# acerbilab/vbmc

Measured on AMD Instinct MI355X. Metric: ELBO+grad evals/sec (Ns=1e4, K=50, D=10, N=400), higher is better.
Workload: dtype f64; 1 GPU; BASELINE configs[2]: D=10 N=400 K=50 Ns=10000/component S=20, R=64 restarts batched per GPU per step, value+gradient, beta=0, no variance; restarts_per_gpu=64, parallelism=one GPU

## Files before the change

vbmc_amd/csrc/entropy_mfma.h:

```cpp
#pragma once
#include <type_traits>

#include "device_math.h"
#include "elbo_types.h"
#include "exp2_tab1k.h"
#include "logjoint_body.h"

typedef double mf4 __attribute__((ext_vector_type(4)));
struct EntTileAny { static constexpr bool rt = false, val = true; };
struct EntTileFull { static constexpr bool rt = false, val = false; };
struct EntTilePartial { static constexpr bool rt = false, val = true; };
#define VBMC_ENT_SPLIT(KT_, QS_, TL_, HV_) ((HV_) == 1)

#ifdef VBMC_INSTRUMENT
#define VBMC_DBG_WAVES 32768
__device__ unsigned long long g_ent_dbg[6 * VBMC_DBG_WAVES];
#endif

#define VBMC_STAG_FOR(KT_, QS_, TL_) ((KT_) == 1 || (KT_) == 4 || ((KT_) == 2 && (QS_) >= 6) || ((KT_) == 3 && (QS_) <= ((TL_) ? 5 : 8)))



constexpr bool ent_c2_for(int KT, int QS, int TL, int HV) {
  if (HV == 1) {
    if (KT == 2) return !(TL == 1 && QS >= 6);
    if (KT == 3) return QS <= 5 || (TL == 0 && QS != 7) || (TL == 1 && QS == 7);
    if (KT == 4) return QS >= 5;
    return true;
  }
  if (HV == 2) {
    if (KT == 2) return TL != 2;
    if (KT == 3) return !((TL == 1 && (QS == 5 || QS == 6)) || (TL == 2 && QS == 6));
    return true;
  }
  if (KT == 2) return !((TL == 1 && QS >= 6) || (TL == 2 && QS >= 5));
  if (KT == 3) return !(TL == 1 && QS == 7);
  return QS != 5;
}
constexpr bool ent_gp2_for(int KT, int QS, int TL, int HV) { return !(HV == 1 && KT == 1 && TL == 0 && QS <= 3); }
constexpr bool ent_sl_for(int KT, int QS, int TL, int HV, bool GRAD, bool WALK) {
  if (!(GRAD && HV == 1 && QS <= 3) || KT == 4 || WALK) return false;
  if (QS == 3) return !((KT == 1 && TL == 0) || (KT == 2 && TL <= 1));
  if (QS == 2) return KT == 3 || (KT == 2 && TL == 0);
  return TL == 0 || (KT == 2 && TL == 1) || (KT == 3 && TL == 2);
}
constexpr bool ent_sl_evl_for(int KT, int QS, int TL) { return QS == 3 && KT == 3 && TL == 0; }

template <int HV>
__device__ __forceinline__ void ent_sync() {
  __builtin_amdgcn_fence(__ATOMIC_RELEASE, "wavefront");
  __builtin_amdgcn_wave_barrier();
  __builtin_amdgcn_fence(__ATOMIC_ACQUIRE, "wavefront");
}
template <int HV>
__device__ __forceinline__ void ent_sync_wg() {
  if (HV == 1) ent_sync<1>();
  else __syncthreads();
}

template <int QS, int KT, bool GRAD, bool SPARSE, int HV = 1, int TL = 0, bool CO = false, bool EM = true, bool WALK = false>
#define VBMC_ENT_EO(HV_) true
#define VBMC_ENT_ONE_WAVE(KT_, QS_, TL_, HV_) \
  (((HV_) == 1 && (KT_) == 4 && (QS_) >= 5) || ((HV_) == 1 && (KT_) == 3 && (QS_) >= 8) || ((HV_) == 4 && (KT_) == 4 && (QS_) >= 6) || \
   ((HV_) == 4 && (KT_) == 3 && (QS_) >= 9))
#define VBMC_ENT_WAVES(KT_, QS_, TL_, HV_) \
  (VBMC_ENT_ONE_WAVE(KT_, QS_, TL_, HV_) ? 1 : ((((KT_) <= 2 && (QS_) <= 4) && !((KT_) == 2 && (TL_) == 2 && (HV_) == 1)) ? 3 : 2))
__device__ __forceinline__ void ent_mfma_segment(const EntArgs& a, const int c, const int j, const int r, const int t0, const int t1,
                                                 const int pdone, const int ptot) {
  static_assert(!CO || (HV == 1 && QS <= 8 && !SPARSE), "the log-joint role exists for single-wave dense kernels at D <= 30");
  static_assert(!WALK || (HV == 1 && !CO), "the walk exists for single-wave workgroups without the log-joint role");
  static_assert(KT <= 4 && (HV == 1 || HV == 2 || HV == 4 || HV == 8), "larger mixtures are split over the waves of a workgroup (HV = 2, 4; round 5: 8, K <= 512)");
  static_assert(TL == 0 || ((TL == 1 || TL == 2) && !SPARSE), "the component tail (one or two values per lane) exists for the dense kernels only");
  constexpr int TLN = TL > 0 ? TL : 1;
  constexpr bool SP = SPARSE;
  constexpr int DP = 4 * QS;
  constexpr int NPV = (4 * QS + 15) / 16;
  constexpr int QL = QS;
  __shared__ double Et[16 * DP];
  constexpr bool SL = NPV == 1 && ent_sl_for(KT, QS, TL, HV, GRAD, WALK);
  constexpr bool GP2 = GRAD && !SL && ent_gp2_for(KT, QS, TL, HV);
  __shared__ double RQ_all[HV][SL ? 1 : (GP2 ? 32 : 16)];
  __shared__ double BND_all[HV][SPARSE ? KT * 16 * 3 : 1];
  constexpr int YXN = NPV * 4 * WAVE;
  constexpr bool EO = VBMC_ENT_EO(HV);
  constexpr bool YXSB = HV > 1 && EO;
  constexpr bool US = EO;
  constexpr bool VBL = GRAD && HV == 1 && (KT >= 3 || NPV >= 2);
  __shared__ double VBS_all[HV][VBL ? KT * 4 * NPV * WAVE : 1];
  constexpr bool C2 = EO && !SPARSE && ent_c2_for(KT, QS, TL, HV);
#define ENT_CI(kt_, rr_) (16 * (kt_) + 4 * (rr_) + lg)
  __shared__ __attribute__((aligned(16))) double SCP_all[HV][C2 ? KT * 16 * 2 : 2];
  __shared__ double BTL_all[HV][TL ? 4 * TL * DP : 1];
  constexpr bool NML = HV > 1 && EO;
  __shared__ double NMS_all[HV][NML ? KT * 4 * WAVE : 1];
#ifdef VBMC_INSTRUMENT
  const unsigned long long wckE = wall_clock64();
#endif
  int tid_ = threadIdx.x;
  if (WALK) asm volatile("" : "+v"(tid_));
  const int tid = tid_, wv = tid >> 6, hv = HV == 1 ? 0 : wv, lane = tid & 63;
  const int li = lane & 15, lg = lane >> 4;
  int D_ = a.D, K_ = a.K;
  const double *entp_ = a.entp, *vpd_ = a.vpd;
  double* part_ = a.part;
  if (WALK) asm volatile("" : "+s"(D_), "+s"(K_), "+s"(entp_), "+s"(vpd_), "+s"(part_));
  const int D = D_, K = K_;
  double* RQ = RQ_all[wv];
  double* NMS = NMS_all[wv];
  double* BND = BND_all[hv];
  double* VBS = VBS_all[hv];
  double* BTL = BTL_all[hv];
  double* SCP = SCP_all[hv];
  const int Kh = (K + HV - 1) / HV;
  const int kbase = hv * Kh;
  const int Kw = min(K, kbase + Kh) - kbase;
  const int PSg = D + ENTP_EXTRA;
  extern __shared__ double PB[];
  double* const TAB = PB;
  double* const YX = PB + VB_EXP_TAB1K_N;
  constexpr int NTH0 = WAVE * HV;
  constexpr int NTB0 = (VB_EXP_TAB1K_N + NTH0 - 1) / NTH0;
  double tt[NTB0];
#pragma unroll
  for (int u = 0; u < NTB0; ++u) tt[u] = c_exp2_tab1k[min(tid + u * NTH0, VB_EXP_TAB1K_N - 1)];
  const double sigj = vpd_[(size_t)r * VpLayout{D, K}.stride() + VpLayout{D, K}.sigma() + j];
  {
    const double* gsrc = entp_ + (size_t)r * K * PSg;
    constexpr int NT = WAVE * HV;
    const int n = K * PSg;
    int idx = tid;
    for (; idx + 7 * NT < n; idx += 8 * NT) {
      double t8[8];
#pragma unroll
      for (int u = 0; u < 8; ++u) t8[u] = gsrc[idx + u * NT];
#pragma unroll
      for (int u = 0; u < 8; ++u) PB[idx + u * NT] = t8[u];
    }
    {
      double t8[8];
#pragma unroll
      for (int u = 0; u < 8; ++u) t8[u] = (idx + u * NT < n) ? gsrc[idx + u * NT] : 0.0;
#pragma unroll
      for (int u = 0; u < 8; ++u) if (idx + u * NT < n) PB[idx + u * NT] = t8[u];
    }
  }
  __syncthreads();
  const double* gp = PB;
  const double* pj = gp + (size_t)j * PSg;
  const double cKj = pj[D + 1];
  const double hj_neg = 0.5 / (sigj * sigj);
  const int nr_last = TL ? 4 : max(1, min(4, (Kw - 16 * (KT - 1) + 3) >> 2));
  constexpr unsigned FULL_MASK = (1u << KT) - 1u;
  const double logwj = SPARSE ? log(pj[D + 2]) : 0.0;

  constexpr double ESC = VB_EXP_TAB1K_SCALE;
  double SA[KT][QL];
  double SC[KT];
  double VB[VBL ? 1 : KT][4][NPV];
  double WF[KT][4];
#pragma unroll
  for (int kt = 0; kt < KT; ++kt) {
    const int k = 16 * kt + li;
    const bool kv = k < Kw;
    const double* pk = gp + (size_t)(kv ? kbase + k : 0) * PSg;
    double h = pk[D];
    double m2 = 0.0;
    for (int d = 0; d < D; ++d) { double t = pk[d] - pj[d]; m2 = fma(t, t, m2); }
    if (SPARSE && lg == 0) {
      BND[(16 * kt + li) * 3 + 0] = sqrt(m2);
      BND[(16 * kt + li) * 3 + 1] = kv ? pk[D + 1] - cKj : -1.0e30;
      BND[(16 * kt + li) * 3 + 2] = h;
    }
#pragma unroll
    for (int q = 0; q < QL; ++q) {
      const int cc = 4 * q + lg;
      if (EO) {
        double sav = (kv && cc < D) ? ESC * (-2.0 * h * (pk[cc] - pj[cc])) : 0.0;
        if (C2) {
          if (cc == D) sav = kv ? ESC * (h + hj_neg) : 0.0;
          if (cc == D + 1) sav = ESC * (kv ? fma(h, m2, pk[D + 1]) - cKj : -1.0e6);
        }
        SA[kt][q] = sav;
      } else {
        double v;
        if (!kv) v = (cc == D + 1) ? -1.0e6 : 0.0;
        else if (cc < D) v = -2.0 * h * (pk[cc] - pj[cc]);
        else if (cc == D) v = h + hj_neg;
        else if (cc == D + 1) v = fma(h, m2, pk[D + 1]) - cKj;
        else v = 0.0;
        SA[kt][q] = ESC * v;
      }
    }
    SC[kt] = ESC * (!kv ? (lg == 1 ? -1.0e6 : 0.0)
                        : (lg == 0 ? h + hj_neg : (lg == 1 ? fma(h, m2, pk[D + 1]) - cKj : 0.0)));
    if (C2 && lg < 2) SCP[(16 * kt + li) * 2 + lg] = 2.0 * SC[kt];
#pragma unroll
    for (int rr = 0; rr < 4; ++rr) {
      const int k2 = ENT_CI(kt, rr);
      const bool kv2 = k2 < Kw;
      const double* p2 = gp + (size_t)(kv2 ? kbase + k2 : 0) * PSg;
      if (GRAD) {
#pragma unroll
        for (int pv = 0; pv < NPV; ++pv) {
          const int col = 16 * pv + li;
          double v = 0.0;
          if (SL) {
            if (kv2) {
              if (li >= 12) v = p2[D + 2];
              else if (li >= 10) v = p2[D + 3];
              else if (li < D) v = p2[D + 3] * (p2[li] - pj[li]);
            }
          } else
          if (kv2) {
            if (col == 0) v = p2[D + 2];
            else if (col == 1) v = p2[D + 3];
            else if (col < 2 + D) v = p2[D + 3] * (p2[col - 2] - pj[col - 2]);
          }
          if (VBL) VBS[((kt * 4 + rr) * NPV + pv) * WAVE + lane] = v;
          else VB[VBL ? 0 : kt][rr][pv] = v;
        }
      } else {
        WF[kt][rr] = kv2 ? p2[D + 2] : 0.0;
      }
    }
  }

  double tC0[TLN], tC1[TLN], VBt[TLN][NPV], WFt[TLN], Wt[TLN];
#pragma unroll
  for (int u = 0; u < TLN; ++u) {
    tC0[u] = 0.0; tC1[u] = 0.0; WFt[u] = 0.0; Wt[u] = 0.0;
#pragma unroll
    for (int pv = 0; pv < NPV; ++pv) VBt[u][pv] = 0.0;
  }
  if (TL) {
#pragma unroll
    for (int u = 0; u < TLN; ++u) {
      const int tq = 4 * u + lg;
      const int kq = 16 * KT + tq;
      const bool kvq = kq < Kw;
      const double* pq = gp + (size_t)(kvq ? kbase + kq : 0) * PSg;
      const double h = pq[D];
      double m2 = 0.0;
      for (int d = 0; d < D; ++d) { double t = pq[d] - pj[d]; m2 = fma(t, t, m2); }
      tC0[u] = kvq ? ESC * (h + hj_neg) : 0.0;
      tC1[u] = ESC * (kvq ? fma(h, m2, pq[D + 1]) - cKj : -1.0e6);
      for (int d = li; d < DP; d += 16) BTL[tq * DP + d] = (kvq && d < D) ? ESC * (-2.0 * h * (pq[d] - pj[d])) : 0.0;
      if (GRAD) {
#pragma unroll
        for (int pv = 0; pv < NPV; ++pv) {
          const int col = 16 * pv + li;
          double v = 0.0;
          if (SL) {
            if (kvq) {
              if (li >= 12) v = pq[D + 2];
              else if (li >= 10) v = pq[D + 3];
              else if (li < D) v = pq[D + 3] * (pq[li] - pj[li]);
            }
          } else
          if (kvq) {
            if (col == 0) v = pq[D + 2];
            else if (col == 1) v = pq[D + 3];
            else if (col < 2 + D) v = pq[D + 3] * (pq[col - 2] - pj[col - 2]);
          }
          VBt[u][pv] = v;
        }
      } else {
        WFt[u] = kvq ? pq[D + 2] : 0.0;
      }
    }
  }

  __syncthreads();
  {
#pragma unroll
    for (int u = 0; u < NTB0; ++u) if (VB_EXP_TAB1K_N % NTH0 == 0 || tid + u * NTH0 < VB_EXP_TAB1K_N) TAB[tid + u * NTH0] = tt[u];
  }
  __syncthreads();

#define SAV(kt_, q_) SA[kt_][q_]
  constexpr int VBR = (VBL && NPV == 1 && HV == 1 && KT == 3 && !CO) ? ((EM && QS <= 4) ? (TL == 2 ? 4 : 10) : 12) : 0;
  double VBreg[VBR > 0 ? VBR : 1];
#pragma unroll
  for (int u = 0; u < VBR; ++u) VBreg[u] = VBS[u * WAVE + lane];
#define VBV(kt_, rr_, pv_) (VBL ? (((kt_) * 4 + (rr_)) * NPV + (pv_) < VBR ? VBreg[(((kt_) * 4 + (rr_)) * NPV + (pv_)) < VBR ? (((kt_) * 4 + (rr_)) * NPV + (pv_)) : 0] : VBS[(((kt_) * 4 + (rr_)) * NPV + (pv_)) * WAVE + lane]) : VB[VBL ? 0 : (kt_)][rr_][pv_])
  constexpr int NG = SL ? QS : NPV;
  double accH = 0.0, accG[NG], accLG[NG];
  double pm = 1.0;
  int pe = 0, pcnt = 0;
  double Wacc[KT][4];
#pragma unroll
  for (int pv = 0; pv < NG; ++pv) { accG[pv] = 0.0; accLG[pv] = 0.0; }
#pragma unroll
  for (int kt = 0; kt < KT; ++kt)
#pragma unroll
    for (int rr = 0; rr < 4; ++rr) Wacc[kt][rr] = 0.0;

#ifdef VBMC_INSTRUMENT
  const unsigned long long wck0 = wall_clock64();
#endif
  const int ntile = (a.Mh + 15) >> 4;
  const double sfm0 = lg == 0 ? 1.0 : 0.0, sfm1 = lg == 1 ? 1.0 : 0.0;
  const int emask = (4 * (QS - 1) + lg < D) ? -1 : 0;
  const int emask2 = (QS >= 2 && 4 * (QS - 2) + lg < D) ? -1 : 0;
  const double* epsr = a.eps ? a.eps + (size_t)r * a.eps_stride_r + (size_t)j * a.Mh * D : nullptr;
  constexpr bool EPF = EM && HV == 1 && QS <= 4 && KT <= 3 && !SPARSE;
  double epre[EPF ? QS : 1];
  auto eps_fetch = [&](const int tile) {
#pragma unroll
    for (int u = 0; u < (EPF ? QS : 0); ++u) {
      const int idx = lane + u * WAVE, i = idx / DP, d = idx - i * DP;
      double v = 0.0;
      if (tile < t1 && d < D && tile * 16 + i < a.Mh) v = epsr[(size_t)(tile * 16 + i) * D + d];
      epre[u] = v;
    }
  };
  if (EPF && epsr) eps_fetch(t0);
  if (!epsr && (HV == 1 || hv == 0))
    for (int idx = lane; idx < 16 * DP; idx += WAVE) Et[idx] = 0.0;
  const int evm1 = emask, evm2 = emask2;
  const double c2u1 = (4 * (QS - 1) + lg == D) ? 1.0 : 0.0, c2o1 = (4 * (QS - 1) + lg == D + 1) ? 1.0 : 0.0;
  const double c2u2 = (QS >= 2 && 4 * (QS - 2) + lg == D) ? 1.0 : 0.0;

  auto tile_body = [&](const int tile, auto pkind) __attribute__((always_inline)) {
    using PK = decltype(pkind);
    const int b0 = tile * 16;
    ent_sync_wg<HV>();
    if (HV > 1 && hv != 0) {
    } else if (EPF && epsr) {
#pragma unroll
      for (int u = 0; u < (EPF ? QS : 0); ++u) Et[lane + u * WAVE] = US ? sigj * epre[u] : epre[u];
      eps_fetch(tile + 1);
    } else if (epsr) {
      for (int idx = lane; idx < 16 * DP; idx += WAVE) {
        const int i = idx / DP, d = idx - i * DP;
        Et[idx] = (d < D && b0 + i < a.Mh) ? (US ? sigj * epsr[(size_t)(b0 + i) * D + d] : epsr[(size_t)(b0 + i) * D + d]) : 0.0;
      }
    } else {
      unsigned long long seed_t = a.seed;
      if (WALK) asm volatile("" : "+s"(seed_t));
#pragma unroll
      for (int q = lg; q < QS; q += 4) {
        double z4[4] = {0.0, 0.0, 0.0, 0.0};
#define VBMC_RNG_CALL_FOR(KT_, QS_, TL_, HV_) ((HV_) == 2 && (((KT_) == 2 && (TL_) == 2 && (QS_) == 5) || ((KT_) == 3 && (TL_) == 0 && (QS_) == 7)))
        if constexpr (!VBMC_RNG_CALL_FOR(KT, QS, TL, HV)) {
        if (q < (D + 3) / 4) { const vb_d4 zz = vb_normal4i(seed_t, (unsigned)(b0 + li), (unsigned)j, (unsigned)(a.r0 + r * a.rstride), (unsigned)q); z4[0] = zz[0]; z4[1] = zz[1]; z4[2] = zz[2]; z4[3] = zz[3]; }
        } else {
        if (q < (D + 3) / 4) vb_normal4(seed_t, (unsigned)(b0 + li), (unsigned)j, (unsigned)(a.r0 + r * a.rstride), (unsigned)q, z4);
        }
#undef VBMC_RNG_CALL_FOR
        if (q < (D + 3) / 4) {
#pragma unroll
        for (int t = 0; t < 4; ++t) Et[li * DP + 4 * q + t] = US ? sigj * z4[t] : z4[t];
        }
      }
    }
    ent_sync_wg<HV>();
    double ev[QS];
    double e2 = 0.0;
#pragma unroll
    for (int q = 0; q < QS; ++q) {
      ev[q] = Et[li * DP + 4 * q + lg];
      if (q == QS - 1) ev[q] = __hiloint2double(__double2hiint(ev[q]) & evm1, __double2loint(ev[q]) & evm1);
      if (QS >= 2 && q == QS - 2) ev[q] = __hiloint2double(__double2hiint(ev[q]) & evm2, __double2loint(ev[q]) & evm2);
      e2 = fma(ev[q], ev[q], e2);
    }
    e2 = xor_sum16(e2);
    e2 = xor_sum32(e2);
    double shift = US ? fma(-e2, hj_neg, cKj) : cKj - 0.5 * e2;
    const double u2 = US ? e2 : sigj * sigj * e2;
    if (US && SPARSE) e2 *= 2.0 * hj_neg;
    constexpr bool partial = PK::val;
    const bool svalid = b0 + li < a.Mh;
    if (partial) shift = svalid ? shift : 0.0;
    unsigned act = FULL_MASK;
    if (SPARSE) {
      double e2m = e2;
      e2m = fmax(e2m, __shfl_xor(e2m, 1, 64)); e2m = fmax(e2m, __shfl_xor(e2m, 2, 64));
      e2m = fmax(e2m, __shfl_xor(e2m, 4, 64)); e2m = fmax(e2m, __shfl_xor(e2m, 8, 64));
      const double umax = sigj * sqrt(e2m);
      const double own = 0.5 * e2m - logwj;
      act = 0u;
#pragma unroll
      for (int kt = 0; kt < KT; ++kt) {
        const double* bk = BND + (16 * kt + li) * 3;
        const double t = fmax(0.0, bk[0] - umax);
        const double bnd = fma(bk[2] * t, t, bk[1]) + own;
        if (__any(bnd > -a.cutoff)) act |= 1u << kt;
      }
    }

    mf4 n[KT], nm[(EO && !NML) ? KT : 1];
    if (EO) {
      const double sfc = fma(u2, sfm0, sfm1);
      double sfl[QL];
#pragma unroll
      for (int q = 0; q < QL; ++q) sfl[q] = US ? ev[q] : ev[q] * sigj;
      if (C2) {
        sfl[QL - 1] = fma(u2, c2u1, sfl[QL - 1] + c2o1);
        if (QS >= 2) sfl[QL >= 2 ? QL - 2 : 0] = fma(u2, c2u2, sfl[QL >= 2 ? QL - 2 : 0]);
      }
#pragma unroll
      for (int kt = 0; kt < KT; ++kt) {
        n[kt] = (mf4){0.0, 0.0, 0.0, 0.0};
        if (!NML) nm[(EO && !NML) ? kt : 0] = (mf4){0.0, 0.0, 0.0, 0.0};
        if (C2) {
#pragma unroll
          for (int q = 0; q < QL; ++q) n[kt] = __builtin_amdgcn_mfma_f64_16x16x4f64(SAV(kt, q), sfl[q], n[kt], 0, 0, 0);
          mf4 e2nd;
#pragma unroll
          for (int rr = 0; rr < 4; ++rr) {
            const double2 pr = *reinterpret_cast<const double2*>(SCP + ENT_CI(kt, rr) * 2);
            e2nd[rr] = fma(pr.x, u2, pr.y) - n[kt][rr];
          }
          if (NML) {
#pragma unroll
            for (int rr = 0; rr < 4; ++rr) NMS[(kt * 4 + rr) * WAVE + lane] = e2nd[rr];
          } else {
            nm[(EO && !NML) ? kt : 0] = e2nd;
          }
        } else
        if (!SP || ((act >> kt) & 1u)) {
          const mf4 cacc = __builtin_amdgcn_mfma_f64_16x16x4f64(SC[kt], sfc, n[kt], 0, 0, 0);
          n[kt] = cacc;
#pragma unroll
          for (int q = 0; q < QL; ++q)
            n[kt] = __builtin_amdgcn_mfma_f64_16x16x4f64(SAV(kt, q), sfl[q], n[kt], 0, 0, 0);
          if (NML) {
            const mf4 e2nd = 2.0 * cacc - n[kt];
#pragma unroll
            for (int rr = 0; rr < 4; ++rr) NMS[(kt * 4 + rr) * WAVE + lane] = e2nd[rr];
          } else {
            nm[(EO && !NML) ? kt : 0] = 2.0 * cacc - n[kt];
          }
        }
      }
    }

    double ntl[TLN], ntm[TLN];
#pragma unroll
    for (int u = 0; u < TLN; ++u) { ntl[u] = 0.0; ntm[u] = 0.0; }
    if (TL) {
#pragma unroll
      for (int u = 0; u < TLN; ++u) {
        double lt = 0.0;
#pragma unroll
        for (int d = 0; d < DP; ++d) lt = fma(BTL[(4 * u + lg) * DP + d], Et[li * DP + d], lt);
        if (!US) lt *= sigj;
        const double ct = fma(tC0[u], u2, tC1[u]);
        ntl[u] = ct + lt;
        ntm[u] = ct - lt;
      }
    }

    auto exps = [&](mf4 (&x)[KT], auto k0c, auto k1c) {
      constexpr int k0 = decltype(k0c)::value, k1 = decltype(k1c)::value;
#pragma unroll
      for (int kt = k0; kt < k1; ++kt) {
        if (kt < KT - 1) {
          if (!SP || ((act >> kt) & 1u)) x[kt] = vb_exp_tab1k4<VB_EXP_TAB1K_QUAD>(x[kt], TAB);
          else x[kt] = (mf4){0.0, 0.0, 0.0, 0.0};
        } else if (SP && !((act >> (KT - 1)) & 1u)) {
          x[KT - 1] = (mf4){0.0, 0.0, 0.0, 0.0};
        } else if (nr_last == 4) {
          x[KT - 1] = vb_exp_tab1k4<VB_EXP_TAB1K_QUAD>(x[KT - 1], TAB);
        } else {
          mf4 t = x[KT - 1];
          x[KT - 1] = (mf4){0.0, 0.0, 0.0, 0.0};
          x[KT - 1][0] = vb_exp_tab1k<VB_EXP_TAB1K_QUAD>(t[0], TAB);
          if (nr_last > 1) x[KT - 1][1] = vb_exp_tab1k<VB_EXP_TAB1K_QUAD>(t[1], TAB);
          if (nr_last > 2) x[KT - 1][2] = vb_exp_tab1k<VB_EXP_TAB1K_QUAD>(t[2], TAB);
        }
      }
    };
    auto texp = [&](double (&t)[TLN]) {
      if (TL) {
#pragma unroll
        for (int u = 0; u < TLN; ++u) t[u] = vb_exp_tab1k<VB_EXP_TAB1K_QUAD>(t[u], TAB);
      }
    };
    auto pvstep = [&](mf4 (&x)[KT], mf4 (&Y)[NPV], int sg, const double (&tn)[TLN]) {
      constexpr bool TWO = NPV == 1 && KT <= 2;
      auto pvm = [&](double xa, double vb, mf4 acc) __attribute__((always_inline)) {
        return SL ? __builtin_amdgcn_mfma_f64_16x16x4f64(vb, xa, acc, 0, 0, 0) : __builtin_amdgcn_mfma_f64_16x16x4f64(xa, vb, acc, 0, 0, 0);
      };
      mf4 Y2s[TWO ? NPV : 1];
      mf4 (&Y2)[TWO ? NPV : 1] = Y2s;
#pragma unroll
      for (int pv = 0; pv < NPV; ++pv) { Y[pv] = (mf4){0.0, 0.0, 0.0, 0.0}; if (TWO) Y2[pv] = (mf4){0.0, 0.0, 0.0, 0.0}; }
#pragma unroll
      for (int kt = 0; kt < KT - 1; ++kt) {
        if (SP && !((act >> kt) & 1u)) continue;
#pragma unroll
        for (int pv = 0; pv < NPV; ++pv) {
          mf4& Yb = TWO ? Y2[TWO ? pv : 0] : Y[pv];
          Y[pv] = pvm(x[kt][0], VBV(kt, 0, pv), Y[pv]);
          Yb = pvm(x[kt][1], VBV(kt, 1, pv), Yb);
          Y[pv] = pvm(x[kt][2], VBV(kt, 2, pv), Y[pv]);
          Yb = pvm(x[kt][3], VBV(kt, 3, pv), Yb);
        }
      }
#pragma unroll
      for (int pv = 0; pv < NPV; ++pv) {
        mf4& Yb = TWO ? Y2[TWO ? pv : 0] : Y[pv];
        if (SP && !((act >> (KT - 1)) & 1u)) { if (TWO) Y[pv] += Yb; continue; }
        Y[pv] = pvm(x[KT - 1][0], VBV(KT - 1, 0, pv), Y[pv]);
        if (nr_last > 1) Yb = pvm(x[KT - 1][1], VBV(KT - 1, 1, pv), Yb);
        if (nr_last > 2) Y[pv] = pvm(x[KT - 1][2], VBV(KT - 1, 2, pv), Y[pv]);
        if (nr_last > 3) Yb = pvm(x[KT - 1][3], VBV(KT - 1, 3, pv), Yb);
        if (TL) {
#pragma unroll
          for (int u = 0; u < TLN; ++u) Y[pv] = pvm(tn[u], VBt[u][pv], Y[pv]);
        }
        if (TWO) Y[pv] += Yb;
      }
      if (HV > 1) {
        if (YXSB && sg == 1) __syncthreads();
#pragma unroll
        for (int pv = 0; pv < NPV; ++pv)
#pragma unroll
          for (int rr = 0; rr < 4; ++rr) YX[((YXSB ? 0 : sg) * HV + hv) * YXN + (pv * 4 + rr) * WAVE + lane] = Y[pv][rr];
        __syncthreads();
#pragma unroll
        for (int pv = 0; pv < NPV; ++pv)
#pragma unroll
          for (int rr = 0; rr < 4; ++rr) {
            double t = YX[((YXSB ? 0 : sg) * HV + 0) * YXN + (pv * 4 + rr) * WAVE + lane];
#pragma unroll
            for (int w = 1; w < HV; ++w) t += YX[((YXSB ? 0 : sg) * HV + w) * YXN + (pv * 4 + rr) * WAVE + lane];
            Y[pv][rr] = t;
          }
      }
    };
    auto put_q = [&](mf4 (&Y)[NPV]) {
      if constexpr (SL) return;
      if (GP2 ? li < 2 : li == 0) {
#pragma unroll
        for (int rr = 0; rr < 4; ++rr) RQ[(GP2 ? 16 * li : 0) + lg + 4 * rr] = Y[0][rr];
      }
      ent_sync<HV>();
    };
    double arq = 0.0;
    constexpr bool TQ = GP2 && US && NPV == 1 && HV == 1 && EO && KT == 3 && QS <= 3 && !CO && !EM && VBMC_STAG_FOR(KT, QS, TL);
    double tq[TQ ? 4 : 1];
    auto get_rq = [&](mf4 (&Y)[NPV]) -> double {
      double qs_ = SL ? Y[0][3] : RQ[li];
      double rqs = vb_rcp(qs_);
      if (partial) {
        qs_ = svalid ? qs_ : 1.0;
        rqs = svalid ? rqs : 0.0;
      }
      if (GP2) arq = RQ[GP2 ? 16 + li : 0] * rqs;
      if (SL) {
        const double t = Y[0][2] * rqs;
        const auto lo = __builtin_amdgcn_permlane32_swap((unsigned)__double2loint(t), (unsigned)__double2loint(t), false, false);
        const auto hi = __builtin_amdgcn_permlane32_swap((unsigned)__double2hiint(t), (unsigned)__double2hiint(t), false, false);
        arq = __hiloint2double((int)hi[1], (int)lo[1]);
      }
      pm *= __builtin_amdgcn_frexp_mant(qs_);
      pe += __builtin_amdgcn_frexp_exp(qs_);
      accH += shift;
      return rqs;
    };
    auto wacc = [&](mf4 (&x)[KT], double rqs, const double (&tn)[TLN]) {
      if (TL) {
#pragma unroll
        for (int u = 0; u < TLN; ++u) Wt[u] = fma(tn[u], rqs, Wt[u]);
      }
#pragma unroll
      for (int kt = 0; kt < KT; ++kt) {
        if (SP && !((act >> kt) & 1u)) continue;
#pragma unroll
        for (int rr = 0; rr < 4; ++rr) Wacc[kt][rr] = fma(x[kt][rr], rqs, Wacc[kt][rr]);
      }
    };
    auto put_rq = [&](double rqs) {
      if constexpr (SL) return;
      ent_sync<HV>();
      if (lg == 0) { RQ[li] = rqs; if (GP2) RQ[GP2 ? 16 + li : 0] = arq; }
      ent_sync<HV>();
    };
    auto gradpieces = [&](mf4 (&Y)[NPV], double rqs, double ssig, auto sgc) {
      constexpr int SG = decltype(sgc)::value;
      constexpr bool EVL = SL && ent_sl_evl_for(KT, QS, TL);
      int eo = li * DP + lg;
      if (EVL) asm volatile("" : "+v"(eo));
      if constexpr (SL) {
#pragma unroll
        for (int r = 0; r < QS; ++r) {
          const double tv = EVL ? Et[eo + 4 * r] : ev[r];
          const double t = (US && SG > 0) ? tv : ((US && SG < 0) ? -tv : ssig * tv);
          const double gd = fma(t, arq, -(Y[0][r] * rqs));
          accG[r] += gd;
          accLG[r] = fma(t, gd, accLG[r]);
        }
        return;
      }
      if constexpr (GP2) {
#pragma unroll
        for (int rr = 0; rr < 4; ++rr) {
          const int i = lg + 4 * rr;
          const double rq = RQ[i], ar = RQ[GP2 ? 16 + i : 0];
#pragma unroll
          for (int pv = 0; pv < NPV; ++pv) {
            if (HV > 1 && (pv % HV) != hv) continue;
            const int d = min(max(16 * pv + li - 2, 0), DP - 1);
            double tv;
            if (TQ) { if (SG >= 0) tq[TQ ? rr : 0] = Et[i * DP + d]; tv = tq[TQ ? rr : 0]; }
            else tv = Et[i * DP + d];
            const double t = (US && SG > 0) ? tv : ((US && SG < 0) ? -tv : ssig * tv);
            const double gd = fma(t, ar, -(Y[pv][rr] * rq));
            accG[pv] += gd;
            accLG[pv] = fma(t, gd, accLG[pv]);
          }
        }
        ent_sync<HV>();
        return;
      }
      const int base = lane & 48;
#pragma unroll
      for (int rr = 0; rr < 4; ++rr) {
        const int i = lg + 4 * rr;
        const double Av = __shfl(Y[0][rr], base | 1, 64);
        const double rq = RQ[i];
#pragma unroll
        for (int pv = 0; pv < NPV; ++pv) {
          if (HV > 1 && (pv % HV) != hv) continue;
          const int d = 16 * pv + li - 2;
          if (d >= 0 && d < D) {
            const double t = (US && SG > 0) ? Et[i * DP + d] : ((US && SG < 0) ? -Et[i * DP + d] : ssig * Et[i * DP + d]);
            const double gd = (t * Av - Y[pv][rr]) * rq;
            accG[pv] += gd;
            accLG[pv] = fma(t, gd, accLG[pv]);
          }
        }
      }
      ent_sync<HV>();
    };
    auto fold = [&]() {
      if (++pcnt == 256) {
        pe += __builtin_amdgcn_frexp_exp(pm);
        pm = __builtin_amdgcn_frexp_mant(pm);
        pcnt = 0;
      }
    };
    using I0 = std::integral_constant<int, 0>;
    using IH = std::integral_constant<int, (KT + 1) / 2>;
    using IK = std::integral_constant<int, KT>;

    if constexpr (EO && GRAD && HV == 1 && VBMC_STAG_FOR(KT, QS, TL)) {
      mf4 Y[NPV];
      exps(n, I0{}, IK{});
      texp(ntl);
      pvstep(n, Y, 0, ntl);
      put_q(Y);
      exps(nm, I0{}, IH{});
      const double rqs = get_rq(Y);
      put_rq(rqs);
      exps(nm, IH{}, IK{});
      texp(ntm);
      wacc(n, rqs, ntl);
      gradpieces(Y, rqs, sigj, std::integral_constant<int, 1>{});
      fold();
      pvstep(nm, Y, 1, ntm);
      put_q(Y);
      const double rqs2 = get_rq(Y);
      wacc(nm, rqs2, ntm);
      put_rq(rqs2);
      gradpieces(Y, rqs2, -sigj, std::integral_constant<int, -1>{});
      fold();
    } else {
      int sg = 0;
      double ssig = US ? 1.0 : sigj;
#pragma unroll 1
      for (;;) {
        if (!EO) {
          double sf[QS];
#pragma unroll
          for (int q = 0; q < QS; ++q) {
            const int cc = 4 * q + lg;
            constexpr bool EVREG = KT <= 3 && QS <= 7;
            sf[q] = (cc < D) ? ssig * (EVREG ? ev[q] : Et[li * DP + 4 * q + lg]) : ((cc == D) ? u2 : ((cc == D + 1) ? 1.0 : 0.0));
          }
#pragma unroll
          for (int kt = 0; kt < KT; ++kt) {
            n[kt] = (mf4){0.0, 0.0, 0.0, 0.0};
#pragma unroll
            for (int q = 0; q < QS; ++q) n[kt] = __builtin_amdgcn_mfma_f64_16x16x4f64(SA[kt][q], sf[q], n[kt], 0, 0, 0);
          }
        }
        exps(n, I0{}, IK{});
        texp(ntl);
        if (GRAD) {
          mf4 Y[NPV];
          pvstep(n, Y, sg, ntl);
          put_q(Y);
          const double rqs = get_rq(Y);
          wacc(n, rqs, ntl);
          put_rq(rqs);
          gradpieces(Y, rqs, ssig, std::integral_constant<int, 0>{});
        } else {
          double qp = 0.0;
#pragma unroll
          for (int kt = 0; kt < KT; ++kt)
#pragma unroll
            for (int rr = 0; rr < 4; ++rr) qp = fma(WF[kt][rr], n[kt][rr], qp);
          if (TL) {
#pragma unroll
            for (int u = 0; u < TLN; ++u) qp = fma(WFt[u], ntl[u], qp);
          }
          qp += __shfl_xor(qp, 16, 64);
          qp += __shfl_xor(qp, 32, 64);
          if (HV > 1) {
            if (YXSB && sg == 1) __syncthreads();
            YX[((YXSB ? 0 : sg) * HV + hv) * YXN + lane] = qp;
            __syncthreads();
            qp = YX[((YXSB ? 0 : sg) * HV + 0) * YXN + lane];
#pragma unroll
            for (int w = 1; w < HV; ++w) qp += YX[((YXSB ? 0 : sg) * HV + w) * YXN + lane];
          }
          double qs_ = qp;
          if (partial) qs_ = svalid ? qp : 1.0;
          pm *= __builtin_amdgcn_frexp_mant(qs_);
          pe += __builtin_amdgcn_frexp_exp(qs_);
          accH += shift;
        }
        fold();
        if (sg) break;
        sg = 1;
        ssig = US ? -1.0 : -sigj;
        if (EO) {
#pragma unroll
          for (int kt = 0; kt < KT; ++kt) {
            if (NML) {
#pragma unroll
              for (int rr = 0; rr < 4; ++rr) n[kt][rr] = NMS[(kt * 4 + rr) * WAVE + lane];
            } else {
              n[kt] = nm[(EO && !NML) ? kt : 0];
            }
          }
        }
#pragma unroll
        for (int u = 0; u < TLN; ++u) ntl[u] = ntm[u];
      }
    }
  };
  if constexpr (VBMC_ENT_SPLIT(KT, QS, TL, HV)) {
    const int tf = min(t1, a.Mh >> 4);
    constexpr bool PRIO = CO ? QS <= 4 : VBMC_ENT_WAVES(KT, QS, TL, HV) > 1;
    const bool pr = PRIO && a.prio != 0;
    const int q1 = pr ? t0 + (ptot + 3) / 4 - pdone : -1, q2 = pr ? t0 + (ptot + 1) / 2 - pdone : -1, q3 = pr ? t0 + (3 * ptot + 3) / 4 - pdone : -1;
    if (pr && pdone == 0) __builtin_amdgcn_s_setprio(3);
    for (int tile = t0; tile < tf; ++tile) {
      if (tile == q1) __builtin_amdgcn_s_setprio(2);
      if (tile == q2) __builtin_amdgcn_s_setprio(1);
      if (tile == q3) __builtin_amdgcn_s_setprio(0);
      tile_body(tile, EntTileFull{});
    }
    if (tf < t1) tile_body(tf, EntTilePartial{});
  } else {
    for (int tile = t0; tile < t1; ++tile) tile_body(tile, EntTileAny{});
  }
#ifdef VBMC_INSTRUMENT
  const unsigned long long wck1 = wall_clock64();
#endif
  if (WALK) accH += vb_log_pos(pm, &pe) + 0.693147180559945309417 * (double)pe;
  else accH += log(pm) + 0.693147180559945309417 * (double)pe;
  if (lg != 0) accH = 0.0;

  double* o = part_ + (((size_t)r * K + j) * a.C + c) * a.ncol;
  accH = wave_sum(accH);
  if (lane == 0 && hv == 0) o[0] = accH;
  if (GRAD) {
    double sgsum = 0.0;
    if constexpr (SL) {
#pragma unroll
      for (int r = 0; r < QS; ++r) {
        double g = accG[r], lgd = accLG[r] / sigj;
        g += __shfl_xor(g, 1, 64); g += __shfl_xor(g, 2, 64);
        g += __shfl_xor(g, 4, 64); g += __shfl_xor(g, 8, 64);
        lgd += __shfl_xor(lgd, 1, 64); lgd += __shfl_xor(lgd, 2, 64);
        lgd += __shfl_xor(lgd, 4, 64); lgd += __shfl_xor(lgd, 8, 64);
        const int d = 4 * r + lg;
        const bool dv = li == 0 && d < D;
        if (dv) { o[1 + d] = g; o[2 + D + d] = lgd; }
        sgsum += dv ? lgd : 0.0;
      }
    } else {
#pragma unroll
    for (int pv = 0; pv < NPV; ++pv) {
      double g = accG[pv], lgd = accLG[pv] / sigj;
      g += __shfl_xor(g, 16, 64); g += __shfl_xor(g, 32, 64);
      lgd += __shfl_xor(lgd, 16, 64); lgd += __shfl_xor(lgd, 32, 64);
      const int d = 16 * pv + li - 2;
      const bool dv = d >= 0 && d < D;
      const bool mine = HV == 1 || (pv % HV) == hv;
      if (dv && lg == 0 && mine) { o[1 + d] = g; o[2 + D + d] = lgd; }
      sgsum += (dv && lg == 0 && mine) ? lgd : 0.0;
    }
    }
    sgsum = wave_sum(sgsum);
    if (HV > 1) {
      __syncthreads();
      if (lane == 0) YX[hv * YXN] = sgsum;
      __syncthreads();
      sgsum = YX[0];
#pragma unroll
      for (int w = 1; w < HV; ++w) sgsum += YX[w * YXN];
    }
    if (lane == 0 && hv == 0) o[1 + D] = sgsum;
#pragma unroll
    for (int kt = 0; kt < KT; ++kt)
#pragma unroll
      for (int rr = 0; rr < 4; ++rr) {
        double wv = Wacc[kt][rr];
        wv += __shfl_xor(wv, 1, 64); wv += __shfl_xor(wv, 2, 64);
        wv += __shfl_xor(wv, 4, 64); wv += __shfl_xor(wv, 8, 64);
        const int k = ENT_CI(kt, rr);
        if (li == 0 && k < Kw) o[2 + 2 * D + kbase + k] = wv;
      }
    if (TL) {
#pragma unroll
      for (int u = 0; u < TLN; ++u) {
        double wv = Wt[u];
        wv += __shfl_xor(wv, 1, 64); wv += __shfl_xor(wv, 2, 64);
        wv += __shfl_xor(wv, 4, 64); wv += __shfl_xor(wv, 8, 64);
        const int k = 16 * KT + 4 * u + lg;
        if (li == 0 && k < Kw) o[2 + 2 * D + kbase + k] = wv;
      }
    }
  }
#ifdef VBMC_INSTRUMENT
  if (lane == 0) {
    const size_t w = ((size_t)r * K + j) * a.C + c;
    if (w < VBMC_DBG_WAVES) {
      g_ent_dbg[6 * w + 0] = wckE; g_ent_dbg[6 * w + 1] = wck0; g_ent_dbg[6 * w + 2] = wck1; g_ent_dbg[6 * w + 3] = wall_clock64();
      g_ent_dbg[6 * w + 4] = __builtin_amdgcn_s_getreg(63492);
      g_ent_dbg[6 * w + 5] = __builtin_amdgcn_s_getreg(63508);
    }
  }
#endif
#undef VBV
#undef SAV
#undef ENT_CI
}

template <int QS, int KT, bool GRAD, bool SPARSE, int HV = 1, int TL = 0, bool CO = false, bool EM = true, bool WALK = false>
__global__ void __launch_bounds__(WAVE * HV, CO ? (QS <= 4 ? 2 : 1) : VBMC_ENT_WAVES(KT, QS, TL, HV)) k_entropy_mfma(EntArgs a) {
  const int ntile = (a.Mh + 15) >> 4;
  constexpr bool walk = WALK;
  int c = (int)blockIdx.x, j = CO ? (int)blockIdx.y - a.lj.rows : (int)blockIdx.y, r = (int)blockIdx.z;
  int tlo = ((int)blockIdx.x + a.c0) * a.tiles_per_chunk, thi = min(tlo + a.tiles_per_chunk, ntile), pdone = 0, rem = 0;
  if (!WALK && a.co_c2 > 0 && c >= a.co_c1) {
    tlo = a.co_c1 * a.tiles_per_chunk + (c - a.co_c1) * a.co_tpc2;
    thi = min(tlo + a.co_tpc2, ntile);
  }
  if (CO) {
    if ((int)blockIdx.y < a.lj.rows) {
      extern __shared__ double PB[];
      lj_co_role<4 * QS>(a.lj, a.vpd, PB);
      const int e = (int)(blockIdx.y * gridDim.x + blockIdx.x);
      if (a.co_c2 <= 0 || e >= a.K * a.co_c2) return;
      j = e / a.co_c2;
      c = a.co_c1 + (e - j * a.co_c2);
      tlo = a.co_c1 * a.tiles_per_chunk + (c - a.co_c1) * a.co_tpc2;
      thi = min(tlo + a.co_tpc2, ntile);
      __syncthreads();
    }
  }
  if (walk) {
    const int g = (int)blockIdx.x * a.walk_tpw;
    rem = min(a.walk_tpw, a.K * a.walk_R * ntile - g);
    const int p = g / ntile;
    tlo = g - p * ntile;
    r = p / a.K;
    j = p - r * a.K;
    c = (int)blockIdx.x - (g - tlo) / a.walk_tpw;
  }
  const int ptot = walk ? rem : thi - tlo;
  for (;;) {
    if (walk) thi = min(ntile, tlo + rem);
    ent_mfma_segment<QS, KT, GRAD, SPARSE, HV, TL, CO, EM, WALK>(a, c, j, r, tlo, thi, pdone, ptot);
    if (!walk) break;
    pdone += thi - tlo;
    rem -= thi - tlo;
    if (rem <= 0) break;
    if (++j == a.K) { j = 0; ++r; }
    tlo = 0;
    c = 0;
    __syncthreads();
  }
}
```

Measured before the change: 31440 evals/s.

## Add paired-sample entropy gradient path for KT=3 QS=3 single-tail kernel

Adds a specialized PM path for the KT=3, QS=3, TL=1 single-wave gradient configuration (D=10, K=50). It processes the plus and minus samples together, computing the weighted mixture sums directly with FMAs against component weights staged in shared memory instead of running the staggered MFMA pvstep sequence twice. The mean-gradient term is then recovered through a per-wave correction subtracted at output time. This cuts per-sample MFMA and reduction work but adds cross-lane reductions and a permlane swap, and it reorganizes the gradient algebra, which carries a numerical-correctness risk.

```diff
diff --git a/vbmc_amd/csrc/entropy_mfma.h b/vbmc_amd/csrc/entropy_mfma.h
--- a/vbmc_amd/csrc/entropy_mfma.h
+++ b/vbmc_amd/csrc/entropy_mfma.h
@@ -45,6 +45,9 @@
   return TL == 0 || (KT == 2 && TL == 1) || (KT == 3 && TL == 2);
 }
 constexpr bool ent_sl_evl_for(int KT, int QS, int TL) { return QS == 3 && KT == 3 && TL == 0; }
+constexpr bool ent_pm_for(int KT, int QS, int TL, int HV, bool GRAD, bool WALK) {
+  return ent_sl_for(KT, QS, TL, HV, GRAD, WALK) && QS == 3 && KT == 3 && TL == 1;
+}
 
 template <int HV>
 __device__ __forceinline__ void ent_sync() {
@@ -79,6 +82,7 @@
   __shared__ double Et[16 * DP];
   constexpr bool SL = NPV == 1 && ent_sl_for(KT, QS, TL, HV, GRAD, WALK);
   constexpr bool GP2 = GRAD && !SL && ent_gp2_for(KT, QS, TL, HV);
+  constexpr bool PM = SL && !SPARSE && ent_pm_for(KT, QS, TL, HV, GRAD, WALK);
   __shared__ double RQ_all[HV][SL ? 1 : (GP2 ? 32 : 16)];
   __shared__ double BND_all[HV][SPARSE ? KT * 16 * 3 : 1];
   constexpr int YXN = NPV * 4 * WAVE;
@@ -91,6 +95,7 @@
 #define ENT_CI(kt_, rr_) (16 * (kt_) + 4 * (rr_) + lg)
   __shared__ __attribute__((aligned(16))) double SCP_all[HV][C2 ? KT * 16 * 2 : 2];
   __shared__ double BTL_all[HV][TL ? 4 * TL * DP : 1];
+  __shared__ __attribute__((aligned(16))) double WAP[PM ? KT * 16 * 2 : 2];
   constexpr bool NML = HV > 1 && EO;
   __shared__ double NMS_all[HV][NML ? KT * 4 * WAVE : 1];
 #ifdef VBMC_INSTRUMENT
@@ -194,6 +199,7 @@
     SC[kt] = ESC * (!kv ? (lg == 1 ? -1.0e6 : 0.0)
                         : (lg == 0 ? h + hj_neg : (lg == 1 ? fma(h, m2, pk[D + 1]) - cKj : 0.0)));
     if (C2 && lg < 2) SCP[(16 * kt + li) * 2 + lg] = 2.0 * SC[kt];
+    if (PM && lg < 2) WAP[(16 * kt + li) * 2 + lg] = kv ? pk[D + 2 + lg] : 0.0;
 #pragma unroll
     for (int rr = 0; rr < 4; ++rr) {
       const int k2 = ENT_CI(kt, rr);
@@ -226,9 +232,10 @@
   }
 
   double tC0[TLN], tC1[TLN], VBt[TLN][NPV], WFt[TLN], Wt[TLN];
+  double tA[TLN];
 #pragma unroll
   for (int u = 0; u < TLN; ++u) {
-    tC0[u] = 0.0; tC1[u] = 0.0; WFt[u] = 0.0; Wt[u] = 0.0;
+    tC0[u] = 0.0; tC1[u] = 0.0; WFt[u] = 0.0; Wt[u] = 0.0; tA[u] = 0.0;
 #pragma unroll
     for (int pv = 0; pv < NPV; ++pv) VBt[u][pv] = 0.0;
   }
@@ -264,6 +271,7 @@
           }
           VBt[u][pv] = v;
         }
+        if (PM) { WFt[u] = kvq ? pq[D + 2] : 0.0; tA[u] = kvq ? pq[D + 3] : 0.0; }
       } else {
         WFt[u] = kvq ? pq[D + 2] : 0.0;
       }
@@ -561,6 +569,17 @@
       accH += shift;
       return rqs;
     };
+    auto rq_pm = [&](double qs_) -> double {
+      double rqs = vb_rcp(qs_);
+      if (partial) {
+        qs_ = svalid ? qs_ : 1.0;
+        rqs = svalid ? rqs : 0.0;
+      }
+      pm *= __builtin_amdgcn_frexp_mant(qs_);
+      pe += __builtin_amdgcn_frexp_exp(qs_);
+      accH += shift;
+      return rqs;
+    };
     auto wacc = [&](mf4 (&x)[KT], double rqs, const double (&tn)[TLN]) {
       if (TL) {
 #pragma unroll
@@ -647,6 +666,72 @@
     using IH = std::integral_constant<int, (KT + 1) / 2>;
     using IK = std::integral_constant<int, KT>;
 
+    if constexpr (PM) {
+      exps(n, I0{}, IK{});
+      texp(ntl);
+      double qp = 0.0, qm = 0.0;
+      if (TL) {
+#pragma unroll
+        for (int u = 0; u < TLN; ++u) qp = fma(WFt[u], ntl[u], qp);
+      }
+#pragma unroll
+      for (int kt = 0; kt < KT; ++kt)
+#pragma unroll
+        for (int rr = 0; rr < 4; ++rr) qp = fma(WAP[ENT_CI(kt, rr) * 2], n[kt][rr], qp);
+      qp = xor_sum16(qp);
+      qp = xor_sum32(qp);
+      const double rqp = rq_pm(qp);
+      fold();
+      exps(nm, I0{}, IK{});
+      texp(ntm);
+      if (TL) {
+#pragma unroll
+        for (int u = 0; u < TLN; ++u) qm = fma(WFt[u], ntm[u], qm);
+      }
+#pragma unroll
+      for (int kt = 0; kt < KT; ++kt)
+#pragma unroll
+        for (int rr = 0; rr < 4; ++rr) qm = fma(WAP[ENT_CI(kt, rr) * 2], nm[kt][rr], qm);
+      qm = xor_sum16(qm);
+      qm = xor_sum32(qm);
+      const double rqm = rq_pm(qm);
+      fold();
+      const double nrqm = -rqm;
+      double ap = 0.0;
+      if (TL) {
+#pragma unroll
+        for (int u = 0; u < TLN; ++u) {
+          const double rp = ntl[u] * rqp, x = ntm[u];
+          ntm[u] = fma(x, rqm, rp);
+          ntl[u] = fma(x, nrqm, rp);
+          Wt[u] += ntm[u];
+          ap = fma(tA[u], ntm[u], ap);
+        }
+      }
+#pragma unroll
+      for (int kt = 0; kt < KT; ++kt)
+#pragma unroll
+        for (int rr = 0; rr < 4; ++rr) {
+          const double rp = n[kt][rr] * rqp, x = nm[kt][rr];
+          nm[kt][rr] = fma(x, rqm, rp);
+          n[kt][rr] = fma(x, nrqm, rp);
+          Wacc[kt][rr] += nm[kt][rr];
+          ap = fma(WAP[ENT_CI(kt, rr) * 2 + 1], nm[kt][rr], ap);
+        }
+      mf4 Y[NPV];
+      pvstep(n, Y, 0, ntl);
+      ap = xor_sum16(ap);
+      ap = xor_sum32(ap);
+      const double t2 = Y[0][2];
+      const auto lo = __builtin_amdgcn_permlane32_swap((unsigned)__double2loint(t2), (unsigned)__double2loint(t2), false, false);
+      const auto hi = __builtin_amdgcn_permlane32_swap((unsigned)__double2hiint(t2), (unsigned)__double2hiint(t2), false, false);
+      const double am = __hiloint2double((int)hi[1], (int)lo[1]);
+#pragma unroll
+      for (int r = 0; r < QS; ++r) {
+        accG[r] = fma(ev[r], am, accG[r]);
+        accLG[r] = fma(ev[r], fma(ev[r], ap, -Y[0][r]), accLG[r]);
+      }
+    } else
     if constexpr (EO && GRAD && HV == 1 && VBMC_STAG_FOR(KT, QS, TL)) {
       mf4 Y[NPV];
       exps(n, I0{}, IK{});
@@ -782,7 +867,7 @@
         lgd += __shfl_xor(lgd, 4, 64); lgd += __shfl_xor(lgd, 8, 64);
         const int d = 4 * r + lg;
         const bool dv = li == 0 && d < D;
-        if (dv) { o[1 + d] = g; o[2 + D + d] = lgd; }
+        if (dv) { if (!PM) o[1 + d] = g; o[2 + D + d] = lgd; }
         sgsum += dv ? lgd : 0.0;
       }
     } else {
@@ -808,6 +893,7 @@
       for (int w = 1; w < HV; ++w) sgsum += YX[w * YXN];
     }
     if (lane == 0 && hv == 0) o[1 + D] = sgsum;
+    double corr = 0.0;
 #pragma unroll
     for (int kt = 0; kt < KT; ++kt)
 #pragma unroll
@@ -817,6 +903,7 @@
         wv += __shfl_xor(wv, 4, 64); wv += __shfl_xor(wv, 8, 64);
         const int k = ENT_CI(kt, rr);
         if (li == 0 && k < Kw) o[2 + 2 * D + kbase + k] = wv;
+        if (PM) corr = fma(VBV(kt, rr, 0), wv, corr);
       }
     if (TL) {
 #pragma unroll
@@ -826,6 +913,19 @@
         wv += __shfl_xor(wv, 4, 64); wv += __shfl_xor(wv, 8, 64);
         const int k = 16 * KT + 4 * u + lg;
         if (li == 0 && k < Kw) o[2 + 2 * D + kbase + k] = wv;
+        if (PM) corr = fma(VBt[u][0], wv, corr);
+      }
+    }
+    if constexpr (PM) {
+      corr = xor_sum16(corr);
+      corr = xor_sum32(corr);
+#pragma unroll
+      for (int r = 0; r < QS; ++r) {
+        double g = accG[r];
+        g += __shfl_xor(g, 1, 64); g += __shfl_xor(g, 2, 64);
+        g += __shfl_xor(g, 4, 64); g += __shfl_xor(g, 8, 64);
+        const int d = 4 * r + lg;
+        if (li == d && d < D) o[1 + d] = g - corr;
       }
     }
   }
```

Measured after the change: 33510 evals/s (median of 6 runs). +6.6%, better.
